# leggedrobotics/art_planner

Hardware: AMD Instinct MI355X
Metric: validated states/sec on 400x400@0.04m map (sample + validity check) (higher is better)
Workload: dtype f32; 1 GPU; C2: lazy_prm_star_min_update front end, 400x400@0.04m Perlin terrain (seed 1234) + 12 obstacles, YAML robot, batch sampler + validity checker; map=400x400@0.04, lanes=1

## Files before the change

art_planner_amd/csrc/artp_capi.hip:

```cpp
#include "../../include/artp_c.h"

#include <hip/hip_runtime.h>
#include <hipcub/hipcub.hpp>

#include <cmath>
#include <cstdio>
#include <atomic>
#include <chrono>
#include <cstdlib>
#include <cstring>
#include <mutex>
#include <string>
#include <array>
#include <vector>

#include "pipeline.h"
#include "cost_kernels.h"

using namespace artp;

#define ARTP_FEW_STATES 16
#define ARTP_SVC_MAX_STATES 2
#define FEW_EDGE_S1 0
#define FEW_EDGE_S2 (ARTP_FEW_EDGES * 7 * sizeof(double))
#define FEW_EDGE_LAST_T (2 * ARTP_FEW_EDGES * 7 * sizeof(double))
#define FEW_EDGE_LAST_STATE (FEW_EDGE_LAST_T + ARTP_FEW_EDGES * sizeof(double))
#define FEW_EDGE_AUX (FEW_EDGE_LAST_STATE + ARTP_FEW_EDGES * 7 * sizeof(double))
#define FEW_EDGE_STATUS (FEW_EDGE_AUX + ARTP_FEW_EDGES * sizeof(uint32_t))
#define FEW_EDGE_BLOCK_BYTES (FEW_EDGE_STATUS + ARTP_FEW_EDGES)
#define ARTP_MAX_LANES 4

struct artp_ctx {
  int device = 0;
  hipStream_t own_stream = nullptr;
  hipStream_t stream = nullptr;
  artp_params params{};
  RobotDev robot{};
// ... 49 lines not shown
  bool poll_labels = true;
  bool svc_enabled = false, svc_launched = false;
  hipStream_t svc_stream = nullptr;
  hipEvent_t svc_after_map = nullptr;
  SvcMailbox* svc = nullptr;
  SvcMailbox* svc_dev = nullptr;
  uint32_t svc_seq = 0;
  uint64_t svc_map_version = 0;
  uint64_t svc_launches = 0, svc_requests = 0;
  bool pool_launched = false;
  hipStream_t pool_stream = nullptr;
  hipEvent_t pool_after_map = nullptr;
  EdgeMailbox* pool_mb = nullptr;
  int pool_bar = -1;
  PoolResponse* pool_resp = nullptr;
  PoolResponse* pool_resp_dev = nullptr;
  PoolCtl* pool_ctl = nullptr;
  uint64_t pool_shadow[5][7] = {};
  unsigned pool_wgs = ARTP_POOL_WGS;
  uint32_t pool_seq = 0;
  uint64_t pool_map_version = 0;
  uint64_t pool_launches = 0, pool_requests = 0;
  char* pin_edges_in = nullptr;
  char* pin_edges_in_dev = nullptr;
  char* pin_edges = nullptr;
  char* pin_edges_dev = nullptr;
  FewEdgeSync* d_few_sync = nullptr;
  int* d_error = nullptr;
  unsigned long long* d_count = nullptr;
  void* tmp[8] = {nullptr, nullptr, nullptr, nullptr, nullptr, nullptr, nullptr, nullptr};
  size_t tmp_cap[8] = {0, 0, 0, 0, 0, 0, 0, 0};
  void* cub_tmp = nullptr;
  size_t cub_cap = 0;
  struct lane_state {
    bool init = false;
    hipStream_t own_stream = nullptr, stream = nullptr;
    unsigned long long* d_count = nullptr;
    int* d_error = nullptr;
    void* tmp[8] = {nullptr, nullptr, nullptr, nullptr, nullptr, nullptr, nullptr, nullptr};
    size_t tmp_cap[8] = {0, 0, 0, 0, 0, 0, 0, 0};
    void* cub_tmp = nullptr;
    size_t cub_cap = 0;
  };
  lane_state lanes[ARTP_MAX_LANES];
  int cur_lane = 0;
  bool have_weights = false;
  int cost_net = 0;
  half8* d_convw[5] = {nullptr, nullptr, nullptr, nullptr, nullptr};
  float* d_convb[5] = {nullptr, nullptr, nullptr, nullptr, nullptr};
  float* d_c12 = nullptr;
  unsigned char* d_c12m = nullptr;
  int conv12_mfma = 1;
  half8* d_convw_chunk[3] = {nullptr, nullptr, nullptr};
  half8* d_convw_p32 = nullptr;
  float* d_fc = nullptr;
  char* d_fc_mfma = nullptr;
  int feet_dense = 0;
  double r3_extent_override = 0.0;
  int fc_mfma = 1;
  int fc_selfcheck = -1;
  float fc_selfcheck_err = 0.f;
  half_t* d_act[2] = {nullptr, nullptr};
  size_t act_cap = 0;
  half_t* d_feat = nullptr;
  size_t feat_cap = 0;
  float* d_map_f32 = nullptr;
  size_t map_cap = 0;
  CostMapGeom cost_geom{};
  int feat_h = 0, feat_w = 0;
  int cost_forms[4] = {0, 0, 0, 0};
  bool have_features = false;
  bool cost_fill_holes = false;
  bool cost_fill_telea = false;
  std::string last_error;
  std::string arch;
  std::recursive_mutex mu;
};

namespace {

#define HIP_TRY(ctx, expr)                                                        \
  do {                                                                            \
    hipError_t _e = (expr);                                                       \
    if (_e != hipSuccess) {                                                       \
      (ctx)->last_error = std::string(#expr) + ": " + hipGetErrorString(_e);      \
      return ARTP_ERR_HIP;                                                        \
    }                                                                             \
  } while (0)

int ensure_tmp(artp_ctx* c, int slot, size_t bytes) {
  if (c->tmp_cap[slot] >= bytes) return ARTP_OK;
  if (c->tmp[slot]) HIP_TRY(c, hipFree(c->tmp[slot]));
  c->tmp[slot] = nullptr;
  c->tmp_cap[slot] = 0;
  const size_t want = bytes + bytes / 4 + 256;
  HIP_TRY(c, hipMalloc(&c->tmp[slot], want));
  c->tmp_cap[slot] = want;
  return ARTP_OK;
}

void park_lane(artp_ctx* c) {
  artp_ctx::lane_state& l = c->lanes[c->cur_lane];
  l.init = true;
  l.own_stream = c->own_stream;
  l.stream = c->stream;
  l.d_count = c->d_count;
  l.d_error = c->d_error;
  l.cub_tmp = c->cub_tmp;
  l.cub_cap = c->cub_cap;
  for (int k = 0; k < 8; ++k) {
    l.tmp[k] = c->tmp[k];
    l.tmp_cap[k] = c->tmp_cap[k];
  }
}

void unpark_lane(artp_ctx* c, int lane) {
  const artp_ctx::lane_state& l = c->lanes[lane];
  c->own_stream = l.own_stream;
  c->stream = l.stream;
  c->d_count = l.d_count;
  c->d_error = l.d_error;
  c->cub_tmp = l.cub_tmp;
  c->cub_cap = l.cub_cap;
  for (int k = 0; k < 8; ++k) {
    c->tmp[k] = l.tmp[k];
    c->tmp_cap[k] = l.tmp_cap[k];
  }
  c->cur_lane = lane;
}

int order_after_other_lanes(artp_ctx* c) {
  for (int l = 0; l < ARTP_MAX_LANES; ++l) {
    if (l == c->cur_lane || !c->lanes[l].init) continue;
    if (!c->lane_mark[l]) HIP_TRY(c, hipEventCreateWithFlags(&c->lane_mark[l], hipEventDisableTiming));
    HIP_TRY(c, hipEventRecord(c->lane_mark[l], c->lanes[l].stream));
    HIP_TRY(c, hipStreamWaitEvent(c->stream, c->lane_mark[l], 0));
  }
  return ARTP_OK;
}

int publish_map_write(artp_ctx* c) {
  if (!c->map_written) HIP_TRY(c, hipEventCreateWithFlags(&c->map_written, hipEventDisableTiming));
  HIP_TRY(c, hipEventRecord(c->map_written, c->stream));
  c->map_seen[c->cur_lane] = ++c->map_write_seq;
  return ARTP_OK;
}

int lane_sees_map(artp_ctx* c) {
  if (c->map_seen[c->cur_lane] != c->map_write_seq && c->map_written) {
    HIP_TRY(c, hipStreamWaitEvent(c->stream, c->map_written, 0));
    c->map_seen[c->cur_lane] = c->map_write_seq;
  }
  return ARTP_OK;
}

void fill_robot(artp_ctx* c) {
// ... 97 lines not shown
  return scratch_bytes_per_wave(c->caps_full) + 4 * scratch_bytes_per_wave(c->caps_foot_full);
}

int opt_in_lds(artp_ctx* c, const void* fn, size_t bytes) {
  static std::mutex mu;
  static std::vector<std::pair<std::pair<int, const void*>, int>> set;
  std::lock_guard<std::mutex> lock(mu);
  int* have = nullptr;
  for (auto& e : set)
    if (e.first.first == c->device && e.first.second == fn) have = &e.second;
  if (have && *have >= (int)bytes) return ARTP_OK;
  HIP_TRY(c, hipFuncSetAttribute(fn, hipFuncAttributeMaxDynamicSharedMemorySize, (int)bytes));
  if (have)
    *have = (int)bytes;
  else
    set.push_back({{c->device, fn}, (int)bytes});
  return ARTP_OK;
}

#define ARTP_OPT_IN(c, kernel, bytes)                                                       \
  do {                                                                                      \
    const int _rc = opt_in_lds((c), reinterpret_cast<const void*>(kernel), (bytes));        \
    if (_rc != ARTP_OK) return _rc;                                                         \
  } while (0)

int set_kernel_lds(artp_ctx* c) {
  ARTP_OPT_IN(c, check_boxes_kernel<1>, lds_full(c));
  ARTP_OPT_IN(c, validate_states_kernel<1>, lds_full(c));
  ARTP_OPT_IN(c, plane_stage_kernel<1>, lds_full(c));
  ARTP_OPT_IN(c, validate_few_kernel, lds_few(c));
  ARTP_OPT_IN(c, check_motions_few_kernel, lds_few(c));
  ARTP_OPT_IN(c, validate_service_kernel, lds_few(c));
  ARTP_OPT_IN(c, check_motions_pool_kernel, lds_few(c));
  ARTP_OPT_IN(c, (resolve_boxes_kernel<ARTP_WAVES_PER_BLOCK, 64, 3>), lds_scan(c));
  ARTP_OPT_IN(c, (resolve_boxes_kernel<ARTP_WAVES_PER_BLOCK, 16, 1>), lds_feet(c));
  ARTP_OPT_IN(c, (resolve_boxes_kernel<ARTP_WAVES_PER_BLOCK, 64, 2>), lds_feet_wave(c));
  return ARTP_OK;
}

int grid_full(const artp_ctx* c, size_t tasks) {
  size_t per_cu = (160 * 1024) / (lds_full(c) ? lds_full(c) : 1);
  if (per_cu > 16) per_cu = 16;
  if (per_cu < 1) per_cu = 1;
  size_t g = (size_t)c->n_cus * per_cu;
  if (tasks && tasks < g) g = tasks;
  return (int)(g ? g : 1);
}
int grid_scan(const artp_ctx* c, size_t lds) {
  size_t per_cu = (160 * 1024) / (lds ? lds : 1);
  if (per_cu > 8) per_cu = 8;
  if (per_cu < 1) per_cu = 1;
  return (int)((size_t)c->n_cus * per_cu);
}

unsigned grid_sub(const artp_ctx* c, int per_cu) {
  const unsigned g = (unsigned)c->n_cus * (unsigned)per_cu;
  return (g + ARTP_NSUB - 1) / ARTP_NSUB * ARTP_NSUB;
}

int partner_radius(const artp_ctx* c, int slot) {
  const FieldDev& f = c->field[slot];
  const float* side = slot == 1 ? c->robot.foot : c->robot.torso;
  const double diag = std::sqrt((double)side[0] * side[0] + (double)side[1] * side[1] + (double)side[2] * side[2]);
  const int R = (int)std::ceil(diag / std::fmin((double)f.sample_w, (double)f.sample_d)) + 3;
  return R > 63 ? -1 : R;
}

static void partner_rect_extent(const FieldDev& f, const PartnerRects& pr, int margin, int* max_cells, int* max_rows) {
// ... 148 lines not shown
    }
    t.st = c->stride_buf[slot];
    t.st_off1 = off[1];
    t.st_off2 = off[2];
    hipLaunchKernelGGL(stride_tables_kernel, dim3((off[3] + 255) / 256), dim3(256), 0, c->stream, t.mm, t.fl, t.stride,
                       f.nW, f.nD, off[1], off[2], off[3], c->stride_buf[slot]);
    HIP_TRY(c, hipGetLastError());
  }
  const int rc_partner = pr ? partner_update_end(c, slot, *pr) : build_partner_table_full(c, slot);
  if (rc_partner != ARTP_OK) return rc_partner;
  t.valid = 1;
  return ARTP_OK;
}

int ensure_recs(artp_ctx* c, size_t n) { return ensure_tmp(c, 7, n * sizeof(PoseRec)); }

int launch_validate_pipeline(artp_ctx* c, const double* se3, size_t n, uint8_t* valid, bool recs_ready = false) {
  if (n >= (1ull << 32)) {
    c->last_error = "batch too large (state index is 32 bit)";
    return ARTP_ERR_INVALID_ARG;
  }
  int rc = ensure_recs(c, n);
  if (rc) return rc;
  PoseRec* recs = static_cast<PoseRec*>(c->tmp[7]);
  if (!recs_ready)
    hipLaunchKernelGGL(pose_rec_kernel, dim3((unsigned)((n + 255) / 256)), dim3(256), 0, c->stream, c->field[0], se3, n,
                       recs);
  const size_t per_block_states = 64 * ARTP_CLASSIFY_SUB;
  const size_t n_blocks = (n + per_block_states - 1) / per_block_states;
  const size_t seg_t = ((n_blocks + ARTP_NSUB - 1) / ARTP_NSUB) * per_block_states;
  rc = ensure_tmp(c, 4, 5 * ARTP_NSUB * seg_t * sizeof(PendingBox));
  if (rc) return rc;
  const size_t ctr_bytes = 128 + (size_t)2 * ARTP_NSUB * 128;
  rc = ensure_tmp(c, 5, ctr_bytes + ((5 + 4 + 4) * n + 5 * (size_t)ARTP_NSUB * seg_t) * sizeof(unsigned) + 64);
  if (rc) return rc;
  PipelineQueues q;
  q.q1 = static_cast<PendingBox*>(c->tmp[4]);
  q.counters = static_cast<unsigned long long*>(c->tmp[5]);
  q.sub = q.counters + 16;
  q.seg_t = seg_t;
  q.q2 = reinterpret_cast<unsigned*>(static_cast<char*>(c->tmp[5]) + ctr_bytes);
  q.q3 = q.q2 + 5 * n;
  q.q5 = q.q3 + 4 * n;
  q.q4 = q.q5 + 4 * n;
  q.q6 = q.q4 + 4 * (size_t)ARTP_NSUB * seg_t;
  q.feet_base = (unsigned long long)ARTP_NSUB * seg_t;
  HIP_TRY(c, hipMemsetAsync(q.counters, 0, ctr_bytes, c->stream));
  const size_t per_block = 64 * ARTP_CLASSIFY_SUB;
  hipLaunchKernelGGL(classify_states_kernel, dim3((unsigned)((n + per_block - 1) / per_block)),
                     dim3(ARTP_CLASSIFY_THREADS), 0, c->stream,
                     c->field[0], c->field[1], c->tables[0], c->tables[1], c->geom, c->robot, (const PoseRec*)recs, n,
                     valid, q);
#ifdef ARTP_VARIANTS
  if (c->feet_dense)
    hipLaunchKernelGGL(feet_stream2_kernel<ARTP_STREAM_WAVES>, dim3(grid_sub(c, ARTP_FEET_WAVES_PER_SIMD)), dim3(64 * ARTP_STREAM_WAVES), 0,
                       c->stream, c->field[1], c->robot, q, valid);
  else
#endif
    hipLaunchKernelGGL(feet_stream_kernel<ARTP_STREAM_WAVES>, dim3(grid_sub(c, ARTP_FEET_WAVES_PER_SIMD)), dim3(64 * ARTP_STREAM_WAVES), 0,
                       c->stream, c->field[1], c->robot, q, valid);
  hipLaunchKernelGGL(feet_lane_kernel, dim3((unsigned)c->n_cus * 8), dim3(ARTP_LANE_THREADS), 0, c->stream,
                     c->field[1], c->robot, q, valid);
  {
    const ScratchCaps caps_stream{0, 0, 0, 0};
    const size_t lds_stream = 0;
    hipLaunchKernelGGL((resolve_boxes_kernel<ARTP_WAVES_PER_BLOCK, 64, 0>), dim3(grid_sub(c, ARTP_TORSO_WGS_PER_CU)),
                       dim3(64 * ARTP_WAVES_PER_BLOCK), lds_stream, c->stream, c->field[0], c->robot, q, valid,
                       caps_stream, c->d_error, c->tables[0].valid ? c->tables[0].mm : (const float2*)nullptr);
  }
  hipLaunchKernelGGL((resolve_boxes_kernel<ARTP_WAVES_PER_BLOCK, 64, 3>), dim3(grid_scan(c, lds_scan(c))),
                     dim3(64 * ARTP_WAVES_PER_BLOCK), lds_scan(c), c->stream, c->field[0], c->robot, q, valid,
                     c->caps_scan, c->d_error);
  hipLaunchKernelGGL((resolve_boxes_kernel<ARTP_WAVES_PER_BLOCK, 16, 1>), dim3(grid_scan(c, lds_feet(c))),
                     dim3(64 * ARTP_WAVES_PER_BLOCK), lds_feet(c), c->stream, c->field[1], c->robot, q, valid,
                     c->caps_feet, c->d_error);
  hipLaunchKernelGGL((resolve_boxes_kernel<ARTP_WAVES_PER_BLOCK, 64, 2>), dim3(grid_scan(c, lds_feet_wave(c))),
                     dim3(64 * ARTP_WAVES_PER_BLOCK), lds_feet_wave(c), c->stream, c->field[1], c->robot, q, valid,
                     c->caps_feet_wave, c->d_error);
  hipLaunchKernelGGL(plane_stage_kernel<1>, dim3(grid_full(c, 0)), dim3(64), lds_full(c), c->stream,
                     c->field[0], c->field[1], c->robot, q, valid, c->caps_full, c->d_error);
  HIP_TRY(c, hipGetLastError());
  return ARTP_OK;
}

int check_error_flag(artp_ctx* c) {
  int flag = 0;
  HIP_TRY(c, hipMemcpyAsync(&flag, c->d_error, sizeof(int), hipMemcpyDeviceToHost, c->stream));
  HIP_TRY(c, hipStreamSynchronize(c->stream));
  if (flag) {
    HIP_TRY(c, hipMemsetAsync(c->d_error, 0, sizeof(int), c->stream));
    c->last_error = "a box window exceeded the LDS tile capacity";
    return ARTP_ERR_CAPACITY;
  }
  return ARTP_OK;
}

}

extern "C" {

void artp_params_defaults(artp_params* p) {
  p->torso_length = 1.05; p->torso_width = 0.55; p->torso_height = 0.2;
  p->torso_off_x = 0.0; p->torso_off_y = 0.0; p->torso_off_z = 0.0;
  p->feet_off_x = 0.362; p->feet_off_y = 0.225; p->feet_off_z = -0.525;
  p->reach_x = 0.25; p->reach_y = 0.1; p->reach_z = 0.15;
  p->unknown_space_untraversable = 1;
  p->max_pitch_pert = 10.0 / 180 * M_PI;
  p->max_roll_pert = 3.33 / 180 * M_PI;
  p->sample_from_distribution = 1;
}

void artp_params_yaml(artp_params* p) {
  p->torso_length = 1.31; p->torso_width = 0.65; p->torso_height = 0.3;
// ... 184 lines not shown
    {
      void *pe = nullptr, *ped = nullptr;
      std::vector<FewEdgeSync> armed(ARTP_FEW_EDGES, FewEdgeSync{0xffffffffu, 0u, 0u, {0u}});
      void *pi = nullptr, *pid = nullptr;
      if (hipHostMalloc(&pi, 2 * ARTP_FEW_EDGES * 7 * sizeof(double), hipHostMallocMapped) == hipSuccess &&
          hipHostGetDevicePointer(&pid, pi, 0) == hipSuccess) {
        c->pin_edges_in = static_cast<char*>(pi);
        c->pin_edges_in_dev = static_cast<char*>(pid);
      } else if (pi) {
        (void)hipHostFree(pi);
      }
      if (!c->pin_edges_in ||
          hipHostMalloc(&pe, FEW_EDGE_BLOCK_BYTES, hipHostMallocMapped) != hipSuccess ||
          hipHostGetDevicePointer(&ped, pe, 0) != hipSuccess ||
          hipMalloc(reinterpret_cast<void**>(&c->d_few_sync), ARTP_FEW_EDGES * sizeof(FewEdgeSync)) != hipSuccess ||
          hipMemcpy(c->d_few_sync, armed.data(), ARTP_FEW_EDGES * sizeof(FewEdgeSync), hipMemcpyHostToDevice) != hipSuccess) {
        if (pe) (void)hipHostFree(pe);
        (void)hipHostFree(ps);
        (void)hipHostFree(pl);
        artp_destroy(c);
        return ARTP_ERR_HIP;
      }
      c->pin_edges = static_cast<char*>(pe);
      c->pin_edges_dev = static_cast<char*>(ped);
    }
    c->pin_states = static_cast<double*>(ps);
    c->pin_labels = static_cast<volatile uint8_t*>(pl);
    c->pin_states_dev = static_cast<double*>(psd);
    c->pin_labels_dev = static_cast<uint8_t*>(pld);
    const char* e = std::getenv("ARTP_NO_POLL");
    c->poll_labels = !(e && e[0] == '1');
#ifdef ARTP_VARIANTS
    if (const char* fd = std::getenv("ARTP_FEET_DENSE")) c->feet_dense = fd[0] != '0';
    if (const char* pw = std::getenv("ARTP_POOL_WGS")) {
      const long v = std::strtol(pw, nullptr, 10);
      if (v >= 1 && v <= ARTP_POOL_MAX_WGS) c->pool_wgs = (unsigned)v;
    }
#endif
  }
  fill_robot(c);
  *out = c;
  return ARTP_OK;
}

void artp_destroy(artp_ctx* c) {
  if (!c) return;
  (void)hipSetDevice(c->device);
  svc_stop(c);
  pool_stop(c);
  park_lane(c);
  for (auto& l : c->lanes)
    if (l.init && l.stream) (void)hipStreamSynchronize(l.stream);
  for (int s = 0; s < 2; ++s)
    if (c->field_data[s]) (void)hipFree(c->field_data[s]);
  if (c->sampler_buf) (void)hipFree(c->sampler_buf);
  if (c->sampler_pack) (void)hipFree(c->sampler_pack);
  if (c->rect_stage_host) (void)hipHostFree(c->rect_stage_host);
  if (c->rect_stage_dev) (void)hipFree(c->rect_stage_dev);
  if (c->rect_stage_done) (void)hipEventDestroy(c->rect_stage_done);
  if (c->map_written) (void)hipEventDestroy(c->map_written);
  for (auto& e : c->lane_mark)
    if (e) (void)hipEventDestroy(e);
  for (auto& l : c->lanes) {
    if (!l.init) continue;
    for (int s = 0; s < 8; ++s)
      if (l.tmp[s]) (void)hipFree(l.tmp[s]);
// ... 1282 lines not shown
int artp_check_motions(artp_ctx* c, const double* s1, const double* s2, size_t n, uint8_t* valid) {
  return run_edges_host(c, 0, s1, s2, n, valid, nullptr);
}
int artp_check_motions_last_valid_dev(artp_ctx* c, const double* s1, const double* s2, size_t n, uint8_t* valid,
                                      double* last_valid_t, double* last_valid_se3) {
  if (n && !last_valid_t) return ARTP_ERR_INVALID_ARG;
  return run_edges_dev(c, 0, s1, s2, n, valid, nullptr, last_valid_t, last_valid_se3);
}
int artp_check_motions_last_valid(artp_ctx* c, const double* s1, const double* s2, size_t n, uint8_t* valid,
                                  double* last_valid_t, double* last_valid_se3) {
  if (n && !last_valid_t) return ARTP_ERR_INVALID_ARG;
  return run_edges_host(c, 0, s1, s2, n, valid, nullptr, last_valid_t, last_valid_se3);
}
int artp_check_edges_interp_dev(artp_ctx* c, const double* s1, const double* s2, size_t n,
                                uint8_t* valid, uint32_t* n_interp_out) {
  return run_edges_dev(c, 1, s1, s2, n, valid, n_interp_out);
}
int artp_check_edges_interp(artp_ctx* c, const double* s1, const double* s2, size_t n, uint8_t* valid,
                            uint32_t* n_interp_out) {
  return run_edges_host(c, 1, s1, s2, n, valid, n_interp_out);
}


namespace {
struct Se3Row { double v[7]; };
}

int artp_debug_pipeline_counters(artp_ctx* c, uint64_t out[8]) {
  if (!c || !out) return ARTP_ERR_INVALID_ARG;
  std::lock_guard<std::recursive_mutex> lock(c->mu);
  if (!c->tmp[5]) return ARTP_ERR_NO_MAP;
  HIP_TRY(c, hipSetDevice(c->device));
  uint64_t raw[16 + 2 * ARTP_NSUB * 16];
  HIP_TRY(c, hipMemcpyAsync(raw, c->tmp[5], sizeof(raw), hipMemcpyDeviceToHost, c->stream));
  HIP_TRY(c, hipStreamSynchronize(c->stream));
  for (int k = 0; k < 8; ++k) out[k] = raw[k];
  out[0] = out[4] = out[2] = out[7] = 0;
  for (int s = 0; s < ARTP_NSUB; ++s) {
    out[0] += raw[16 + (size_t)s * 16];
    out[4] += raw[16 + (size_t)(ARTP_NSUB + s) * 16];
    out[2] += raw[16 + (size_t)s * 16 + 2];
    out[7] += raw[16 + (size_t)(ARTP_NSUB + s) * 16 + 2];
  }
  return ARTP_OK;
}

int artp_debug_partner_table(artp_ctx* c, int slot, uint8_t* out, size_t out_bytes, int* radius) {
  if (!c || slot < 0 || slot > 1 || !radius) return ARTP_ERR_INVALID_ARG;
  std::lock_guard<std::recursive_mutex> lock(c->mu);
  if (!c->have_field[slot]) return ARTP_ERR_NO_MAP;
  const FieldDev& f = c->field[slot];
  *radius = f.partner_flags ? f.partner_R : 0;
  if (!out || !f.partner_flags) return ARTP_OK;
  const size_t need = (size_t)f.nW * f.nD;
  if (out_bytes < need) return ARTP_ERR_INVALID_ARG;
  HIP_TRY(c, hipSetDevice(c->device));
  HIP_TRY(c, hipMemcpyAsync(out, f.partner_flags, need, hipMemcpyDeviceToHost, c->stream));
  HIP_TRY(c, hipStreamSynchronize(c->stream));
  return ARTP_OK;
}

int artp_compact_valid_dev(artp_ctx* c, const double* se3, const uint8_t* valid, size_t n,
                           double* out_se3, uint64_t* n_out_dev) {
  if (!c || (n && (!se3 || !valid || !out_se3)) || !n_out_dev) return ARTP_ERR_INVALID_ARG;
  std::lock_guard<std::recursive_mutex> lock(c->mu);
  HIP_TRY(c, hipSetDevice(c->device));
  if (n == 0) {
// ... 1144 lines not shown
  return ARTP_OK;
}

int artp_cost_get_features(artp_ctx* c, float* out, int* fh, int* fw) {
  return artp_cost_get_features_c(c, out, 48, fh, fw);
}

}

#include "roadmap.h"
#include "tree.h"
#include "roadmap_many.h"
#include "reach.h"
#include "preprocess.h"
#include "group.h"

#ifdef ARTP_STAGE_TIMING
extern "C" int artp_debug_few_trace(unsigned long long* out40) {
  return hipMemcpyFromSymbol(out40, HIP_SYMBOL(artp::g_few_trace), 40 * sizeof(unsigned long long)) == hipSuccess ? 0 : -1;
}
extern "C" int artp_debug_pool_trace(unsigned long long* out16) {
  return hipMemcpyFromSymbol(out16, HIP_SYMBOL(artp::g_pool_trace), 16 * sizeof(unsigned long long)) == hipSuccess ? 0 : -1;
}
extern "C" int artp_debug_stage_cycles(unsigned long long* out20, int reset) {
  if (out20 && hipMemcpyFromSymbol(out20, HIP_SYMBOL(artp::g_stage_cycles), 20 * sizeof(unsigned long long)) != hipSuccess)
    return -1;
  if (out20 && reset >= 3 &&
      hipMemcpyFromSymbol(out20, HIP_SYMBOL(artp::g_feet_cycles), 4 * sizeof(unsigned long long)) != hipSuccess)
    return -1;
  if (reset) {
    unsigned long long z4[4] = {};
    if (hipMemcpyToSymbol(HIP_SYMBOL(artp::g_feet_cycles), z4, sizeof(z4)) != hipSuccess) return -1;
  }
  if (reset == 6) {
    return out20 && hipMemcpyFromSymbol(out20, HIP_SYMBOL(artp::g_ks_trace), 1024 * 6 * sizeof(unsigned long long)) == hipSuccess ? 0 : -1;
  }
  if (reset == 5) {
    static unsigned long long all[256 * 12 * 4];
    if (hipMemcpyFromSymbol(all, HIP_SYMBOL(artp::g_kwalk_cycles), sizeof(all)) != hipSuccess) return -1;
    if (out20)
      for (int k = 0; k < 48; ++k) {
        out20[k] = 0;
        for (int b = 0; b < 256; ++b) out20[k] += all[b * 48 + k];
      }
    std::memset(all, 0, sizeof(all));
    return hipMemcpyToSymbol(HIP_SYMBOL(artp::g_kwalk_cycles), all, sizeof(all)) == hipSuccess ? 0 : -1;
  }
  if (reset == 4) {
    if (out20 && hipMemcpyFromSymbol(out20, HIP_SYMBOL(artp::g_cnn_cycles), 16 * sizeof(unsigned long long)) != hipSuccess) return -1;
    unsigned long long z16[16] = {};
    return hipMemcpyToSymbol(HIP_SYMBOL(artp::g_cnn_cycles), z16, sizeof(z16)) == hipSuccess ? 0 : -1;
  }
  if (out20 && reset == 2 &&
      hipMemcpyFromSymbol(out20, HIP_SYMBOL(artp::g_classify_cycles), 16 * sizeof(unsigned long long)) != hipSuccess)
    return -1;
  if (reset) {
    unsigned long long z16[16] = {};
    if (hipMemcpyToSymbol(HIP_SYMBOL(artp::g_classify_cycles), z16, sizeof(z16)) != hipSuccess) return -1;
    unsigned long long z[20] = {};
    if (hipMemcpyToSymbol(HIP_SYMBOL(artp::g_stage_cycles), z, sizeof(z)) != hipSuccess) return -1;
  }
  return 0;
}
#endif
```

art_planner_amd/csrc/pipeline.h:

```cpp
#pragma once

#include <hip/hip_fp16.h>

#include "kernels.h"

namespace artp {

#define ARTP_TABLE_LEVELS 4

struct TablesDev {
  const float2* mm;
  const unsigned char* fl;
  unsigned stride;
  int has_nan;
  int has_nonfinite;
  int valid;
  const unsigned* st;
  unsigned st_off1, st_off2;
};

#define ARTP_STRIDE_LEVELS 3

__global__ void __launch_bounds__(256)
table_level0_kernel(const float* __restrict__ data, int n, float2* __restrict__ mm, unsigned char* __restrict__ fl) {
// ... 772 lines not shown
                         (f_xp_zm && f_xp) || (f_zm && f_xm);
                }
              }
            } else {
              w.allFinite = false;
            }
           }
          }
        }
        int result = 0, ec;
        bool decided = !(rec.kind & ARTP_REC_EXITS_NEGATIVE) && decide_exits(b, w, result, ec);
        if (!decided && vhit) {
          result = 1;
          decided = true;
        }
        if (decided && result == 0) valid[rec.state] = 0;
        undecided = !decided;
      }
    }
    const unsigned long long b3 = __ballot(undecided);
    unsigned long long base3 = 0;
    if (lane == 0 && b3) base3 = atomicAdd(&q.counters[5], (unsigned long long)__popcll(b3));
    base3 = __shfl(base3, 0, 64);
    if (undecided) q.q3[base3 + __popcll(b3 & lt_mask)] = (unsigned)item;
  }
}

#ifdef ARTP_STAGE_TIMING
__device__ unsigned long long g_feet_cycles[4];
#endif
#ifndef ARTP_FEET_WAVES_PER_SIMD
#define ARTP_FEET_WAVES_PER_SIMD 6
#endif
template <int WAVES>
__global__ void __launch_bounds__(64 * WAVES) __attribute__((amdgpu_waves_per_eu(ARTP_FEET_WAVES_PER_SIMD, ARTP_FEET_WAVES_PER_SIMD)))
feet_stream_kernel(FieldDev ff, RobotDev rb, PipelineQueues q, uint8_t* __restrict__ valid) {
  constexpr int G = 16, GPW = 4;
  const int lane = threadIdx.x & 63;
  const int gl = lane & (G - 1);
  const int sq = blockIdx.x % ARTP_NSUB;
  const unsigned long long count = *sub_counter(q, 1, sq);
  const unsigned long long first = sub_base(q, 1, sq);
  unsigned long long* cursor = sub_cursor(q, 1, sq);
  for (;;) {
    unsigned long long chunk = 0;
    if (lane == 0) chunk = atomicAdd(cursor, (unsigned long long)ARTP_FEET_CHUNK);
    chunk = __shfl(chunk, 0);
    if (chunk >= count) break;
    for (int r = 0; r < ARTP_FEET_CHUNK / GPW; ++r) {
      const unsigned long long it = chunk + (unsigned long long)(r * GPW + lane / G);
      if (it < count) {
        const unsigned long long item = first + it;
        const PendingBox rec = q.q1[item];
        if (valid[rec.state] != 0) {
          if (rec.kind & ARTP_REC_EXITS_NEGATIVE) {
            BoxHF b;
            box_from_record(rec, rb, b);
#ifdef ARTP_STAGE_TIMING
            const long long tf0 = clock64();
#endif
            const bool touches = grp_vertex_stream<G, ARTP_FEET_U>(ff, b, lane, (rec.kind & ARTP_REC_ALL_FINITE) != 0);
#ifdef ARTP_STAGE_TIMING
            const long long tf1 = clock64();
            if (gl == 0) atomicAdd(&g_feet_cycles[0], (unsigned long long)(tf1 - tf0));
#endif
            if (!touches) {
              const int rr = grp_corner_stage_direct<G>(ff, b, lane);
#ifdef ARTP_STAGE_TIMING
              if (gl == 0) {
                atomicAdd(&g_feet_cycles[1], (unsigned long long)(clock64() - tf1));
                atomicAdd(&g_feet_cycles[2], 1ull);
              }
#endif
              if (gl == 0) {
                if (rr == 2)
                  q.q5[atomicAdd(&q.counters[6], 1ull)] = (unsigned)item;
                else if (rr == 0)
                  valid[rec.state] = 0;
              }
            }
          }
        }
      }
    }
  }
}



#ifdef ARTP_STAGE_TIMING
__device__ unsigned long long g_stage_cycles[2][10];
#define ARTP_T_MARK(slot)                    \
  do {                                       \
    const long long now_ = clock64();        \
    t_acc[slot] += (unsigned long long)(now_ - t_prev); \
    t_prev = now_;                           \
  } while (0)
#else
#define ARTP_T_MARK(slot) do { } while (0)
#endif

template <int WAVES, int G, int PASS>
__global__ void __launch_bounds__(64 * WAVES)
resolve_boxes_kernel(FieldDev fld, RobotDev rb, PipelineQueues q, uint8_t* __restrict__ valid,
                     ScratchCaps caps, int* __restrict__ error_flag, const float2* __restrict__ mm4 = nullptr) {
  extern __shared__ __attribute__((aligned(16))) char smem[];
  constexpr int GPW = 64 / G;
  const int lane = threadIdx.x & 63;
  const int gl = lane & (G - 1);
  const int unit_in_block = (threadIdx.x >> 6) * GPW + (lane / G);
  const WaveScratch s = carve_scratch(smem, unit_in_block, caps);
  const bool direct = PASS == 1 && fwd_total(q, 1) < ARTP_LANE_SCAN_MIN;
  const bool feet = (PASS == 1 && !direct) || PASS == 2;
  const int sq = blockIdx.x % ARTP_NSUB;
  const unsigned long long count =
      PASS == 0 ? *sub_counter(q, 0, sq)
                : (PASS == 3 ? fwd_total(q, 0) : (direct ? fwd_total(q, 1) : q.counters[PASS == 1 ? 5 : 6]));
  const unsigned long long first = PASS == 0 ? sub_base(q, 0, sq) : 0ull;
  const unsigned long long nblk = PASS == 0 ? gridDim.x / ARTP_NSUB : gridDim.x;
  const unsigned long long blk = PASS == 0 ? blockIdx.x / ARTP_NSUB : blockIdx.x;
  const unsigned long long stride = nblk * WAVES * GPW;
#ifdef ARTP_STAGE_TIMING
  unsigned long long t_acc[8] = {0, 0, 0, 0, 0, 0, 0, 0};
  const long long t_begin = clock64();
#endif
  unsigned long long next = PASS == 0 ? 0ull : blk * WAVES * GPW + unit_in_block, chunk_end = 0ull;
  __shared__ unsigned fwd_slots[PASS == 0 ? WAVES : 1][ARTP_TORSO_CHUNK];
  unsigned* fs = fwd_slots[PASS == 0 ? (threadIdx.x >> 6) : 0];
  if (PASS == 0 && lane < ARTP_TORSO_CHUNK) fs[lane] = 0u;
  unsigned long long chunk_first = 0ull;
  for (;;) {
    if constexpr (PASS == 0) {
      if (next >= chunk_end) {
        fwd_flush_slots<ARTP_TORSO_CHUNK>(fs, sub_fwd(q, 0, sq), q.q6 + fwd_base(q, 0, sq), lane);
        unsigned long long c0 = 0;
        if (lane == 0) c0 = atomicAdd(sub_cursor(q, 0, sq), (unsigned long long)ARTP_TORSO_CHUNK);
        c0 = __shfl(c0, 0);
        if (c0 >= count) break;
        next = c0;
        chunk_first = c0;
        chunk_end = c0 + ARTP_TORSO_CHUNK < count ? c0 + ARTP_TORSO_CHUNK : count;
      }
    } else {
      if (next >= count) break;
    }
    const unsigned long long it = next;
    next += PASS == 0 ? 1ull : stride;
    const unsigned long long item =
        PASS == 0 ? first + it
                  : (unsigned long long)(PASS == 1 ? (direct ? fwd_item(q, 1, q.q4, it) : q.q3[it])
                                                   : (PASS == 2 ? q.q5[it] : fwd_item(q, 0, q.q6, it)));
#ifdef ARTP_STAGE_TIMING
    long long t_prev = clock64();
#endif
    const PendingBox rec = q.q1[item];
    if (valid[rec.state] == 0) continue;
    BoxHF b;
    box_from_record(rec, rb, b);
    ARTP_T_MARK(0);
    int result = 0, ec, fast_r = 2;
    bool decided = false;
    if constexpr (PASS == 0) {
      if (fld.partner_flags != nullptr && (rec.kind & ARTP_REC_ALL_FINITE)) {
        __shared__ unsigned short hot_blocks[WAVES][ARTP_HOT_BLOCKS];
        if (wave_vertex_stream_blocks<ARTP_TORSO_U>(fld, mm4, b, hot_blocks[threadIdx.x >> 6], lane)) {
          result = 1;
          decided = true;
        } else {
          ARTP_T_MARK(2);
          const int r = grp_corner_stage_direct<G>(fld, b, lane);
          if (r != 2) {
            result = r;
            decided = true;
          }
        }
        ARTP_T_MARK(4);
      }
      if (!decided) {
        if (gl == 0) fs[it - chunk_first] = (unsigned)item + 1u;
      } else if (gl == 0 && result != 0) {
        valid[rec.state] = 0;
      }
      continue;
    }
    const int total = (b.maxX - b.minX + 1) * (b.maxZ - b.minZ + 1);
    if (total > s.cap_verts) {
      if (gl == 0) atomicExch(error_flag, 1);
      continue;
    }
    WindowStats w;
    if (!decided) {
      grp_scan_window<G>(fld, b, s, lane, w);
      ARTP_T_MARK(1);
      decided = !feet && decide_exits(b, w, result, ec);
    }
    if (!decided) {
      const bool vhit = !feet && grp_vertex_pass<G>(fld, b, s, lane, w.allFinite);
      ARTP_T_MARK(2);
      if (vhit) {
        result = 1;
        decided = true;
      } else if (PASS == 1) {
        const int r = grp_plane_stage_corners<G>(fld, b, s, lane, 0, true);
        ARTP_T_MARK(4);
        if (r != 2) {
          result = r;
          decided = true;
        } else if (gl == 0) {
          const unsigned long long slot = atomicAdd(&q.counters[6], 1ull);
          q.q5[slot] = (unsigned)item;
        }
      } else if (PASS == 3 && fld.partner_flags != nullptr &&
                 (fast_r = grp_plane_stage_corners<G>(fld, b, s, lane, 0, true)) != 2) {
        ARTP_T_MARK(4);
        result = fast_r;
        decided = true;
      } else {
        const int T = grp_compact_triangles<G, true>(b, s, lane);
        ARTP_T_MARK(3);
#ifdef ARTP_STAGE_TIMING
        const int r = (T == 0) ? 0 : (T < 0 ? 2 : grp_plane_stage_corners<G>(fld, b, s, lane, T, false, t_acc));
#else
        const int r = (T == 0) ? 0 : (T < 0 ? 2 : grp_plane_stage_corners<G>(fld, b, s, lane, T));
#endif
        ARTP_T_MARK(4);
        if (r != 2) {
          result = r;
          decided = true;
        } else if (gl == 0) {
          const unsigned long long slot = atomicAdd(&q.counters[1], 1ull);
          q.q2[slot] = (unsigned)item;
        }
      }
    }
    if (decided && gl == 0) {
      const bool ok = (rec.kind & 1u) ? (result != 0) : (result == 0);
      if (!ok) valid[rec.state] = 0;
    }
    wave_lds_sync();
  }
#ifdef ARTP_STAGE_TIMING
  if (gl == 0) {
    for (int k = 0; k < 8; ++k) atomicAdd(&g_stage_cycles[G == 64 ? 0 : 1][k], t_acc[k]);
    atomicAdd(&g_stage_cycles[G == 64 ? 0 : 1][8], (unsigned long long)(clock64() - t_begin));
    atomicAdd(&g_stage_cycles[G == 64 ? 0 : 1][9], 1ull);
  }
#endif
}

template <int WAVES>
__global__ void __launch_bounds__(64 * WAVES)
plane_stage_kernel(FieldDev fb, FieldDev ff, RobotDev rb, PipelineQueues q, uint8_t* __restrict__ valid,
                   ScratchCaps caps, int* __restrict__ error_flag) {
  extern __shared__ __attribute__((aligned(16))) char smem[];
  const int lane = threadIdx.x & 63;
  const WaveScratch s = carve_scratch(smem, threadIdx.x >> 6, caps);
  const unsigned long long count = q.counters[1];
  const unsigned long long stride = (unsigned long long)gridDim.x * WAVES;
  for (unsigned long long item = (unsigned long long)blockIdx.x * WAVES + (threadIdx.x >> 6); item < count;
       item += stride) {
    const PendingBox rec = q.q1[q.q2[item]];
    if (valid[rec.state] == 0) continue;
    BoxHF b;
    box_from_record(rec, rb, b);
    const bool foot = (rec.kind & 1u) != 0;
    WindowStats w;
    if (foot)
      wave_scan_window(ff, b, s, lane, w);
    else
      wave_scan_window(fb, b, s, lane, w);
    const int T = wave_compact_triangles<true>(b, s, lane);
    int result;
    if (T < 0)
      result = (foot ? wave_plane_stage_unlisted(ff, b, s, lane) : wave_plane_stage_unlisted(fb, b, s, lane)) ? 1 : 0;
    else
      result = (T > 0 && (foot ? wave_plane_stage(ff, b, s, lane, T) : wave_plane_stage(fb, b, s, lane, T))) ? 1 : 0;
    if (lane == 0) {
      const bool ok = (rec.kind & 1u) ? (result != 0) : (result == 0);
      if (!ok) valid[rec.state] = 0;
    }
    wave_lds_sync();
  }
}

#ifdef ARTP_VARIANTS
#include "pipeline_variants.h"
#endif

// ... 2 lines not shown
```

Before: 3.682 billion states/s.

## Double-buffer pipeline counters and merge torso/feet resolve passes into one launch

```diff
diff --git a/art_planner_amd/csrc/artp_capi.hip b/art_planner_amd/csrc/artp_capi.hip
--- a/art_planner_amd/csrc/artp_capi.hip
+++ b/art_planner_amd/csrc/artp_capi.hip
@@ -3,6 +3,7 @@
 #include <hip/hip_runtime.h>
 #include <hipcub/hipcub.hpp>
 
+#include <algorithm>
 #include <cmath>
 #include <cstdio>
 #include <atomic>
@@ -118,6 +119,9 @@
   size_t tmp_cap[8] = {0, 0, 0, 0, 0, 0, 0, 0};
   void* cub_tmp = nullptr;
   size_t cub_cap = 0;
+  int ctr_sel = 0;
+  bool ctr_clean = false;
+  hipStream_t ctr_stream = nullptr;
   struct lane_state {
     bool init = false;
     hipStream_t own_stream = nullptr, stream = nullptr;
@@ -127,6 +131,9 @@
     size_t tmp_cap[8] = {0, 0, 0, 0, 0, 0, 0, 0};
     void* cub_tmp = nullptr;
     size_t cub_cap = 0;
+    int ctr_sel = 0;
+    bool ctr_clean = false;
+    hipStream_t ctr_stream = nullptr;
   };
   lane_state lanes[ARTP_MAX_LANES];
   int cur_lane = 0;
@@ -142,6 +149,7 @@
   float* d_fc = nullptr;
   char* d_fc_mfma = nullptr;
   int feet_dense = 0;
+  int stream_merge = 0;
   double r3_extent_override = 0.0;
   int fc_mfma = 1;
   int fc_selfcheck = -1;
@@ -179,6 +187,7 @@
   if (c->tmp[slot]) HIP_TRY(c, hipFree(c->tmp[slot]));
   c->tmp[slot] = nullptr;
   c->tmp_cap[slot] = 0;
+  if (slot == 5) c->ctr_clean = false;
   const size_t want = bytes + bytes / 4 + 256;
   HIP_TRY(c, hipMalloc(&c->tmp[slot], want));
   c->tmp_cap[slot] = want;
@@ -194,6 +203,9 @@
   l.d_error = c->d_error;
   l.cub_tmp = c->cub_tmp;
   l.cub_cap = c->cub_cap;
+  l.ctr_sel = c->ctr_sel;
+  l.ctr_clean = c->ctr_clean;
+  l.ctr_stream = c->ctr_stream;
   for (int k = 0; k < 8; ++k) {
     l.tmp[k] = c->tmp[k];
     l.tmp_cap[k] = c->tmp_cap[k];
@@ -208,6 +220,9 @@
   c->d_error = l.d_error;
   c->cub_tmp = l.cub_tmp;
   c->cub_cap = l.cub_cap;
+  c->ctr_sel = l.ctr_sel;
+  c->ctr_clean = l.ctr_clean;
+  c->ctr_stream = l.ctr_stream;
   for (int k = 0; k < 8; ++k) {
     c->tmp[k] = l.tmp[k];
     c->tmp_cap[k] = l.tmp_cap[k];
@@ -371,8 +386,7 @@
   ARTP_OPT_IN(c, check_motions_few_kernel, lds_few(c));
   ARTP_OPT_IN(c, validate_service_kernel, lds_few(c));
   ARTP_OPT_IN(c, check_motions_pool_kernel, lds_few(c));
-  ARTP_OPT_IN(c, (resolve_boxes_kernel<ARTP_WAVES_PER_BLOCK, 64, 3>), lds_scan(c));
-  ARTP_OPT_IN(c, (resolve_boxes_kernel<ARTP_WAVES_PER_BLOCK, 16, 1>), lds_feet(c));
+  ARTP_OPT_IN(c, resolve_staged_kernel<ARTP_WAVES_PER_BLOCK>, std::max(lds_scan(c), lds_feet(c)));
   ARTP_OPT_IN(c, (resolve_boxes_kernel<ARTP_WAVES_PER_BLOCK, 64, 2>), lds_feet_wave(c));
   return ARTP_OK;
 }
@@ -587,27 +601,37 @@
   rc = ensure_tmp(c, 4, 5 * ARTP_NSUB * seg_t * sizeof(PendingBox));
   if (rc) return rc;
   const size_t ctr_bytes = 128 + (size_t)2 * ARTP_NSUB * 128;
-  rc = ensure_tmp(c, 5, ctr_bytes + ((5 + 4 + 4) * n + 5 * (size_t)ARTP_NSUB * seg_t) * sizeof(unsigned) + 64);
+  rc = ensure_tmp(c, 5, 2 * ctr_bytes + ((5 + 4 + 4) * n + 5 * (size_t)ARTP_NSUB * seg_t) * sizeof(unsigned) + 64);
   if (rc) return rc;
+  const bool clean = c->ctr_clean && c->ctr_stream == c->stream;
+  const int sel = clean ? c->ctr_sel ^ 1 : 0;
+  c->ctr_clean = false;
   PipelineQueues q;
   q.q1 = static_cast<PendingBox*>(c->tmp[4]);
-  q.counters = static_cast<unsigned long long*>(c->tmp[5]);
+  q.counters = reinterpret_cast<unsigned long long*>(static_cast<char*>(c->tmp[5]) + (size_t)sel * ctr_bytes);
+  unsigned long long* next_counters =
+      reinterpret_cast<unsigned long long*>(static_cast<char*>(c->tmp[5]) + (size_t)(sel ^ 1) * ctr_bytes);
   q.sub = q.counters + 16;
   q.seg_t = seg_t;
-  q.q2 = reinterpret_cast<unsigned*>(static_cast<char*>(c->tmp[5]) + ctr_bytes);
+  q.q2 = reinterpret_cast<unsigned*>(static_cast<char*>(c->tmp[5]) + 2 * ctr_bytes);
   q.q3 = q.q2 + 5 * n;
   q.q5 = q.q3 + 4 * n;
   q.q4 = q.q5 + 4 * n;
   q.q6 = q.q4 + 4 * (size_t)ARTP_NSUB * seg_t;
   q.feet_base = (unsigned long long)ARTP_NSUB * seg_t;
-  HIP_TRY(c, hipMemsetAsync(q.counters, 0, ctr_bytes, c->stream));
+  c->ctr_sel = sel;
+  if (!clean) HIP_TRY(c, hipMemsetAsync(q.counters, 0, ctr_bytes, c->stream));
   const size_t per_block = 64 * ARTP_CLASSIFY_SUB;
   hipLaunchKernelGGL(classify_states_kernel, dim3((unsigned)((n + per_block - 1) / per_block)),
                      dim3(ARTP_CLASSIFY_THREADS), 0, c->stream,
                      c->field[0], c->field[1], c->tables[0], c->tables[1], c->geom, c->robot, (const PoseRec*)recs, n,
                      valid, q);
+  const float2* mm4 = c->tables[0].valid ? c->tables[0].mm : (const float2*)nullptr;
 #ifdef ARTP_VARIANTS
-  if (c->feet_dense)
+  if (c->stream_merge)
+    hipLaunchKernelGGL(stream_boxes_kernel, dim3(grid_sub(c, ARTP_FEET_WAVES_PER_SIMD)), dim3(64 * ARTP_STREAM_WAVES), 0,
+                       c->stream, c->field[0], c->field[1], c->robot, q, valid, mm4);
+  else if (c->feet_dense)
     hipLaunchKernelGGL(feet_stream2_kernel<ARTP_STREAM_WAVES>, dim3(grid_sub(c, ARTP_FEET_WAVES_PER_SIMD)), dim3(64 * ARTP_STREAM_WAVES), 0,
                        c->stream, c->field[1], c->robot, q, valid);
   else
@@ -616,24 +640,30 @@
                        c->stream, c->field[1], c->robot, q, valid);
   hipLaunchKernelGGL(feet_lane_kernel, dim3((unsigned)c->n_cus * 8), dim3(ARTP_LANE_THREADS), 0, c->stream,
                      c->field[1], c->robot, q, valid);
+#ifdef ARTP_VARIANTS
+  if (!c->stream_merge)
+#endif
   {
     const ScratchCaps caps_stream{0, 0, 0, 0};
-    const size_t lds_stream = 0;
     hipLaunchKernelGGL((resolve_boxes_kernel<ARTP_WAVES_PER_BLOCK, 64, 0>), dim3(grid_sub(c, ARTP_TORSO_WGS_PER_CU)),
-                       dim3(64 * ARTP_WAVES_PER_BLOCK), lds_stream, c->stream, c->field[0], c->robot, q, valid,
-                       caps_stream, c->d_error, c->tables[0].valid ? c->tables[0].mm : (const float2*)nullptr);
-  }
-  hipLaunchKernelGGL((resolve_boxes_kernel<ARTP_WAVES_PER_BLOCK, 64, 3>), dim3(grid_scan(c, lds_scan(c))),
-                     dim3(64 * ARTP_WAVES_PER_BLOCK), lds_scan(c), c->stream, c->field[0], c->robot, q, valid,
-                     c->caps_scan, c->d_error);
-  hipLaunchKernelGGL((resolve_boxes_kernel<ARTP_WAVES_PER_BLOCK, 16, 1>), dim3(grid_scan(c, lds_feet(c))),
-                     dim3(64 * ARTP_WAVES_PER_BLOCK), lds_feet(c), c->stream, c->field[1], c->robot, q, valid,
-                     c->caps_feet, c->d_error);
+                       dim3(64 * ARTP_WAVES_PER_BLOCK), 0, c->stream, c->field[0], c->robot, q, valid,
+                       caps_stream, c->d_error, mm4);
+  }
+  {
+    const unsigned n_torso = (unsigned)grid_scan(c, lds_scan(c)), n_feet = (unsigned)grid_scan(c, lds_feet(c));
+    hipLaunchKernelGGL(resolve_staged_kernel<ARTP_WAVES_PER_BLOCK>, dim3(n_torso + n_feet), dim3(64 * ARTP_WAVES_PER_BLOCK),
+                       std::max(lds_scan(c), lds_feet(c)), c->stream, c->field[0], c->field[1], c->robot, q, valid,
+                       c->caps_scan, c->caps_feet, c->d_error, n_torso);
+  }
   hipLaunchKernelGGL((resolve_boxes_kernel<ARTP_WAVES_PER_BLOCK, 64, 2>), dim3(grid_scan(c, lds_feet_wave(c))),
                      dim3(64 * ARTP_WAVES_PER_BLOCK), lds_feet_wave(c), c->stream, c->field[1], c->robot, q, valid,
                      c->caps_feet_wave, c->d_error);
   hipLaunchKernelGGL(plane_stage_kernel<1>, dim3(grid_full(c, 0)), dim3(64), lds_full(c), c->stream,
-                     c->field[0], c->field[1], c->robot, q, valid, c->caps_full, c->d_error);
+                     c->field[0], c->field[1], c->robot, q, valid, c->caps_full, c->d_error, next_counters,
+                     (unsigned)(ctr_bytes / sizeof(unsigned long long)));
+  HIP_TRY(c, hipGetLastError());
+  c->ctr_clean = true;
+  c->ctr_stream = c->stream;
   HIP_TRY(c, hipGetLastError());
   return ARTP_OK;
 }
@@ -884,6 +914,7 @@
     c->poll_labels = !(e && e[0] == '1');
 #ifdef ARTP_VARIANTS
     if (const char* fd = std::getenv("ARTP_FEET_DENSE")) c->feet_dense = fd[0] != '0';
+    if (const char* sm = std::getenv("ARTP_STREAM_MERGE")) c->stream_merge = sm[0] != '0';
     if (const char* pw = std::getenv("ARTP_POOL_WGS")) {
       const long v = std::strtol(pw, nullptr, 10);
       if (v >= 1 && v <= ARTP_POOL_MAX_WGS) c->pool_wgs = (unsigned)v;
@@ -2232,7 +2263,8 @@
   if (!c->tmp[5]) return ARTP_ERR_NO_MAP;
   HIP_TRY(c, hipSetDevice(c->device));
   uint64_t raw[16 + 2 * ARTP_NSUB * 16];
-  HIP_TRY(c, hipMemcpyAsync(raw, c->tmp[5], sizeof(raw), hipMemcpyDeviceToHost, c->stream));
+  HIP_TRY(c, hipMemcpyAsync(raw, static_cast<char*>(c->tmp[5]) + (size_t)c->ctr_sel * sizeof(raw), sizeof(raw),
+                            hipMemcpyDeviceToHost, c->stream));
   HIP_TRY(c, hipStreamSynchronize(c->stream));
   for (int k = 0; k < 8; ++k) out[k] = raw[k];
   out[0] = out[4] = out[2] = out[7] = 0;
@@ -3443,6 +3475,11 @@
     unsigned long long z4[4] = {};
     if (hipMemcpyToSymbol(HIP_SYMBOL(artp::g_feet_cycles), z4, sizeof(z4)) != hipSuccess) return -1;
   }
+  if (reset == 7) {
+    unsigned long long z2[2] = {};
+    if (out20 && hipMemcpyFromSymbol(out20, HIP_SYMBOL(artp::g_torso_stream_boxes), sizeof(z2)) != hipSuccess) return -1;
+    return hipMemcpyToSymbol(HIP_SYMBOL(artp::g_torso_stream_boxes), z2, sizeof(z2)) == hipSuccess ? 0 : -1;
+  }
   if (reset == 6) {
     return out20 && hipMemcpyFromSymbol(out20, HIP_SYMBOL(artp::g_ks_trace), 1024 * 6 * sizeof(unsigned long long)) == hipSuccess ? 0 : -1;
   }
diff --git a/art_planner_amd/csrc/pipeline.h b/art_planner_amd/csrc/pipeline.h
--- a/art_planner_amd/csrc/pipeline.h
+++ b/art_planner_amd/csrc/pipeline.h
@@ -828,13 +828,10 @@
 #ifndef ARTP_FEET_WAVES_PER_SIMD
 #define ARTP_FEET_WAVES_PER_SIMD 6
 #endif
-template <int WAVES>
-__global__ void __launch_bounds__(64 * WAVES) __attribute__((amdgpu_waves_per_eu(ARTP_FEET_WAVES_PER_SIMD, ARTP_FEET_WAVES_PER_SIMD)))
-feet_stream_kernel(FieldDev ff, RobotDev rb, PipelineQueues q, uint8_t* __restrict__ valid) {
+__device__ __forceinline__ void feet_stream_chunks(const FieldDev& ff, const RobotDev& rb, const PipelineQueues& q,
+                                                   uint8_t* __restrict__ valid, int lane, int sq) {
   constexpr int G = 16, GPW = 4;
-  const int lane = threadIdx.x & 63;
   const int gl = lane & (G - 1);
-  const int sq = blockIdx.x % ARTP_NSUB;
   const unsigned long long count = *sub_counter(q, 1, sq);
   const unsigned long long first = sub_base(q, 1, sq);
   unsigned long long* cursor = sub_cursor(q, 1, sq);
@@ -882,6 +879,12 @@
   }
 }
 
+template <int WAVES>
+__global__ void __launch_bounds__(64 * WAVES) __attribute__((amdgpu_waves_per_eu(ARTP_FEET_WAVES_PER_SIMD, ARTP_FEET_WAVES_PER_SIMD)))
+feet_stream_kernel(FieldDev ff, RobotDev rb, PipelineQueues q, uint8_t* __restrict__ valid) {
+  feet_stream_chunks(ff, rb, q, valid, threadIdx.x & 63, blockIdx.x % ARTP_NSUB);
+}
+
 
 
 #ifdef ARTP_STAGE_TIMING
@@ -896,10 +899,101 @@
 #define ARTP_T_MARK(slot) do { } while (0)
 #endif
 
+#ifdef ARTP_STAGE_TIMING
+__device__ unsigned long long g_torso_stream_boxes[2];
+#endif
+__device__ __forceinline__ void torso_stream_chunks(const FieldDev& fld, const RobotDev& rb, const PipelineQueues& q,
+                                                    uint8_t* __restrict__ valid, const float2* __restrict__ mm4,
+                                                    int lane, int sq, unsigned* fs, unsigned short* hot) {
+  constexpr int G = 64;
+  const int gl = lane;
+  const unsigned long long count = *sub_counter(q, 0, sq);
+  const unsigned long long first = sub_base(q, 0, sq);
+#ifdef ARTP_STAGE_TIMING
+  unsigned long long t_acc[8] = {0, 0, 0, 0, 0, 0, 0, 0};
+  const long long t_begin = clock64();
+#endif
+  unsigned long long next = 0ull, chunk_end = 0ull;
+  if (lane < ARTP_TORSO_CHUNK) fs[lane] = 0u;
+  unsigned long long chunk_first = 0ull;
+  for (;;) {
+    if (next >= chunk_end) {
+      fwd_flush_slots<ARTP_TORSO_CHUNK>(fs, sub_fwd(q, 0, sq), q.q6 + fwd_base(q, 0, sq), lane);
+      unsigned long long c0 = 0;
+      if (lane == 0) c0 = atomicAdd(sub_cursor(q, 0, sq), (unsigned long long)ARTP_TORSO_CHUNK);
+      c0 = __shfl(c0, 0);
+      if (c0 >= count) break;
+      next = c0;
+      chunk_first = c0;
+      chunk_end = c0 + ARTP_TORSO_CHUNK < count ? c0 + ARTP_TORSO_CHUNK : count;
+    }
+    const unsigned long long it = next;
+    next += 1ull;
+    const unsigned long long item = first + it;
+#ifdef ARTP_STAGE_TIMING
+    long long t_prev = clock64();
+#endif
+    const PendingBox rec = q.q1[item];
+#ifdef ARTP_STAGE_TIMING
+    if (gl == 0) {
+      atomicAdd(&g_torso_stream_boxes[0], 1ull);
+      if (valid[rec.state] != 0) atomicAdd(&g_torso_stream_boxes[1], 1ull);
+    }
+#endif
+    if (valid[rec.state] == 0) continue;
+    BoxHF b;
+    box_from_record(rec, rb, b);
+    ARTP_T_MARK(0);
+    int result = 0;
+    bool decided = false;
+    if (fld.partner_flags != nullptr && (rec.kind & ARTP_REC_ALL_FINITE)) {
+      if (wave_vertex_stream_blocks<ARTP_TORSO_U>(fld, mm4, b, hot, lane)) {
+        result = 1;
+        decided = true;
+      } else {
+        ARTP_T_MARK(2);
+        const int r = grp_corner_stage_direct<G>(fld, b, lane);
+        if (r != 2) {
+          result = r;
+          decided = true;
+        }
+      }
+      ARTP_T_MARK(4);
+    }
+    if (!decided) {
+      if (gl == 0) fs[it - chunk_first] = (unsigned)item + 1u;
+    } else if (gl == 0 && result != 0) {
+      valid[rec.state] = 0;
+    }
+  }
+#ifdef ARTP_STAGE_TIMING
+  if (gl == 0) {
+    for (int k = 0; k < 8; ++k) atomicAdd(&g_stage_cycles[0][k], t_acc[k]);
+    atomicAdd(&g_stage_cycles[0][8], (unsigned long long)(clock64() - t_begin));
+    atomicAdd(&g_stage_cycles[0][9], 1ull);
+  }
+#endif
+}
+
+#ifdef ARTP_VARIANTS
+__global__ void __launch_bounds__(64 * ARTP_STREAM_WAVES) __attribute__((amdgpu_waves_per_eu(ARTP_FEET_WAVES_PER_SIMD, ARTP_FEET_WAVES_PER_SIMD)))
+stream_boxes_kernel(FieldDev fb, FieldDev ff, RobotDev rb, PipelineQueues q, uint8_t* __restrict__ valid,
+                    const float2* __restrict__ mm4) {
+  __shared__ unsigned fwd_slots[ARTP_STREAM_WAVES][ARTP_TORSO_CHUNK];
+  __shared__ unsigned short hot_blocks[ARTP_STREAM_WAVES][ARTP_HOT_BLOCKS];
+  const int lane = threadIdx.x & 63;
+  const int wave = threadIdx.x >> 6;
+  const int sq = blockIdx.x % ARTP_NSUB;
+  feet_stream_chunks(ff, rb, q, valid, lane, sq);
+  torso_stream_chunks(fb, rb, q, valid, mm4, lane, sq, fwd_slots[wave], hot_blocks[wave]);
+}
+#endif
+
 template <int WAVES, int G, int PASS>
-__global__ void __launch_bounds__(64 * WAVES)
-resolve_boxes_kernel(FieldDev fld, RobotDev rb, PipelineQueues q, uint8_t* __restrict__ valid,
-                     ScratchCaps caps, int* __restrict__ error_flag, const float2* __restrict__ mm4 = nullptr) {
+__device__ __forceinline__ void resolve_boxes_pass(const FieldDev& fld, const RobotDev& rb, const PipelineQueues& q,
+                                                   uint8_t* __restrict__ valid, const ScratchCaps& caps,
+                                                   int* __restrict__ error_flag, unsigned long long blk,
+                                                   unsigned long long nblk) {
   extern __shared__ __attribute__((aligned(16))) char smem[];
   constexpr int GPW = 64 / G;
   const int lane = threadIdx.x & 63;
@@ -908,44 +1002,17 @@
   const WaveScratch s = carve_scratch(smem, unit_in_block, caps);
   const bool direct = PASS == 1 && fwd_total(q, 1) < ARTP_LANE_SCAN_MIN;
   const bool feet = (PASS == 1 && !direct) || PASS == 2;
-  const int sq = blockIdx.x % ARTP_NSUB;
   const unsigned long long count =
-      PASS == 0 ? *sub_counter(q, 0, sq)
-                : (PASS == 3 ? fwd_total(q, 0) : (direct ? fwd_total(q, 1) : q.counters[PASS == 1 ? 5 : 6]));
-  const unsigned long long first = PASS == 0 ? sub_base(q, 0, sq) : 0ull;
-  const unsigned long long nblk = PASS == 0 ? gridDim.x / ARTP_NSUB : gridDim.x;
-  const unsigned long long blk = PASS == 0 ? blockIdx.x / ARTP_NSUB : blockIdx.x;
+      PASS == 3 ? fwd_total(q, 0) : (direct ? fwd_total(q, 1) : q.counters[PASS == 1 ? 5 : 6]);
   const unsigned long long stride = nblk * WAVES * GPW;
 #ifdef ARTP_STAGE_TIMING
   unsigned long long t_acc[8] = {0, 0, 0, 0, 0, 0, 0, 0};
   const long long t_begin = clock64();
 #endif
-  unsigned long long next = PASS == 0 ? 0ull : blk * WAVES * GPW + unit_in_block, chunk_end = 0ull;
-  __shared__ unsigned fwd_slots[PASS == 0 ? WAVES : 1][ARTP_TORSO_CHUNK];
-  unsigned* fs = fwd_slots[PASS == 0 ? (threadIdx.x >> 6) : 0];
-  if (PASS == 0 && lane < ARTP_TORSO_CHUNK) fs[lane] = 0u;
-  unsigned long long chunk_first = 0ull;
-  for (;;) {
-    if constexpr (PASS == 0) {
-      if (next >= chunk_end) {
-        fwd_flush_slots<ARTP_TORSO_CHUNK>(fs, sub_fwd(q, 0, sq), q.q6 + fwd_base(q, 0, sq), lane);
-        unsigned long long c0 = 0;
-        if (lane == 0) c0 = atomicAdd(sub_cursor(q, 0, sq), (unsigned long long)ARTP_TORSO_CHUNK);
-        c0 = __shfl(c0, 0);
-        if (c0 >= count) break;
-        next = c0;
-        chunk_first = c0;
-        chunk_end = c0 + ARTP_TORSO_CHUNK < count ? c0 + ARTP_TORSO_CHUNK : count;
-      }
-    } else {
-      if (next >= count) break;
-    }
-    const unsigned long long it = next;
-    next += PASS == 0 ? 1ull : stride;
+  for (unsigned long long it = blk * WAVES * GPW + unit_in_block; it < count; it += stride) {
     const unsigned long long item =
-        PASS == 0 ? first + it
-                  : (unsigned long long)(PASS == 1 ? (direct ? fwd_item(q, 1, q.q4, it) : q.q3[it])
-                                                   : (PASS == 2 ? q.q5[it] : fwd_item(q, 0, q.q6, it)));
+        (unsigned long long)(PASS == 1 ? (direct ? fwd_item(q, 1, q.q4, it) : q.q3[it])
+                                       : (PASS == 2 ? q.q5[it] : fwd_item(q, 0, q.q6, it)));
 #ifdef ARTP_STAGE_TIMING
     long long t_prev = clock64();
 #endif
@@ -956,29 +1023,6 @@
     ARTP_T_MARK(0);
     int result = 0, ec, fast_r = 2;
     bool decided = false;
-    if constexpr (PASS == 0) {
-      if (fld.partner_flags != nullptr && (rec.kind & ARTP_REC_ALL_FINITE)) {
-        __shared__ unsigned short hot_blocks[WAVES][ARTP_HOT_BLOCKS];
-        if (wave_vertex_stream_blocks<ARTP_TORSO_U>(fld, mm4, b, hot_blocks[threadIdx.x >> 6], lane)) {
-          result = 1;
-          decided = true;
-        } else {
-          ARTP_T_MARK(2);
-          const int r = grp_corner_stage_direct<G>(fld, b, lane);
-          if (r != 2) {
-            result = r;
-            decided = true;
-          }
-        }
-        ARTP_T_MARK(4);
-      }
-      if (!decided) {
-        if (gl == 0) fs[it - chunk_first] = (unsigned)item + 1u;
-      } else if (gl == 0 && result != 0) {
-        valid[rec.state] = 0;
-      }
-      continue;
-    }
     const int total = (b.maxX - b.minX + 1) * (b.maxZ - b.minZ + 1);
     if (total > s.cap_verts) {
       if (gl == 0) atomicExch(error_flag, 1);
@@ -1044,12 +1088,39 @@
 #endif
 }
 
+template <int WAVES, int G, int PASS>
+__global__ void __launch_bounds__(64 * WAVES)
+resolve_boxes_kernel(FieldDev fld, RobotDev rb, PipelineQueues q, uint8_t* __restrict__ valid,
+                     ScratchCaps caps, int* __restrict__ error_flag, const float2* __restrict__ mm4 = nullptr) {
+  if constexpr (PASS == 0) {
+    __shared__ unsigned fwd_slots[WAVES][ARTP_TORSO_CHUNK];
+    __shared__ unsigned short hot_blocks[WAVES][ARTP_HOT_BLOCKS];
+    const int wave = threadIdx.x >> 6;
+    torso_stream_chunks(fld, rb, q, valid, mm4, threadIdx.x & 63, blockIdx.x % ARTP_NSUB, fwd_slots[wave], hot_blocks[wave]);
+  } else {
+    resolve_boxes_pass<WAVES, G, PASS>(fld, rb, q, valid, caps, error_flag, blockIdx.x, gridDim.x);
+  }
+}
+
+template <int WAVES>
+__global__ void __launch_bounds__(64 * WAVES)
+resolve_staged_kernel(FieldDev fb, FieldDev ff, RobotDev rb, PipelineQueues q, uint8_t* __restrict__ valid,
+                      ScratchCaps caps_torso, ScratchCaps caps_feet, int* __restrict__ error_flag, unsigned n_torso) {
+  if (blockIdx.x < n_torso)
+    resolve_boxes_pass<WAVES, 64, 3>(fb, rb, q, valid, caps_torso, error_flag, blockIdx.x, n_torso);
+  else
+    resolve_boxes_pass<WAVES, 16, 1>(ff, rb, q, valid, caps_feet, error_flag, blockIdx.x - n_torso, gridDim.x - n_torso);
+}
+
 template <int WAVES>
 __global__ void __launch_bounds__(64 * WAVES)
 plane_stage_kernel(FieldDev fb, FieldDev ff, RobotDev rb, PipelineQueues q, uint8_t* __restrict__ valid,
-                   ScratchCaps caps, int* __restrict__ error_flag) {
+                   ScratchCaps caps, int* __restrict__ error_flag, unsigned long long* __restrict__ next_counters,
+                   unsigned counter_words) {
   extern __shared__ __attribute__((aligned(16))) char smem[];
   const int lane = threadIdx.x & 63;
+  if (blockIdx.x == 0)
+    for (unsigned i = threadIdx.x; i < counter_words; i += 64 * WAVES) next_counters[i] = 0ull;
   const WaveScratch s = carve_scratch(smem, threadIdx.x >> 6, caps);
   const unsigned long long count = q.counters[1];
   const unsigned long long stride = (unsigned long long)gridDim.x * WAVES;
```

Result: no change. 3.695 billion states/s (median of 6 runs) (+0.4%).
